# argumentcomputer/lurk-beta

Measured on AMD Instinct MI355X. Metric: MSM Mscalar-mul/s (Pallas Pedersen commitment, bases+scalars resident in HBM), higher is better.
Workload: dtype u32x8 (255-bit Montgomery, integer VALU)

## Files before the change

### lurk_beta_amd/csrc/field.cuh

```cuda
#pragma once
#include <stdint.h>

#if defined(__HIPCC__)
#define LURK_HD __host__ __device__ __forceinline__
#else
#define LURK_HD inline
#endif

namespace lurk {

struct PallasFp {
    static constexpr int ID = 0;
    static constexpr int NBITS = 255;
    static constexpr uint32_t INV = 0xffffffffu;
    LURK_HD static constexpr uint32_t mod(int i) {
        constexpr uint32_t m[8] = {0x00000001u, 0x992d30edu, 0x094cf91bu, 0x224698fcu, 0x00000000u, 0x00000000u, 0x00000000u, 0x40000000u};
        return m[i];
    }
    LURK_HD static constexpr uint32_t r(int i) {
        constexpr uint32_t m[8] = {0xfffffffdu, 0x34786d38u, 0xe41914adu, 0x992c350bu, 0xffffffffu, 0xffffffffu, 0xffffffffu, 0x3fffffffu};
        return m[i];
    }
    LURK_HD static constexpr uint32_t r2(int i) {
        constexpr uint32_t m[8] = {0x0000000fu, 0x8c78ecb3u, 0x8b0de0e7u, 0xd7d30dbdu, 0xc3c95d18u, 0x7797a99bu, 0x7b9cb714u, 0x096d41afu};
        return m[i];
    }
    LURK_HD static constexpr uint32_t w32(int i) {
        constexpr uint32_t m[8] = {0xbad6dbf0u, 0xa28db849u, 0xd3b539dfu, 0x9083cd03u, 0x9dc8448eu, 0xfba6b9cau, 0x7b89c6dau, 0x3ec92874u};
        return m[i];
    }
};

struct PallasFq {
    static constexpr int ID = 1;
    static constexpr int NBITS = 255;
    static constexpr uint32_t INV = 0xffffffffu;
    LURK_HD static constexpr uint32_t mod(int i) {
        constexpr uint32_t m[8] = {0x00000001u, 0x8c46eb21u, 0x0994a8ddu, 0x224698fcu, 0x00000000u, 0x00000000u, 0x00000000u, 0x40000000u};
        return m[i];
    }
    LURK_HD static constexpr uint32_t r(int i) {
        constexpr uint32_t m[8] = {0xfffffffdu, 0x5b2b3e9cu, 0xe3420567u, 0x992c350bu, 0xffffffffu, 0xffffffffu, 0xffffffffu, 0x3fffffffu};
        return m[i];
    }
    LURK_HD static constexpr uint32_t r2(int i) {
        constexpr uint32_t m[8] = {0x0000000fu, 0xfc9678ffu, 0x891a16e3u, 0x67bb433du, 0x04ccf590u, 0x7fae2310u, 0x7ccfdaa9u, 0x096d41afu};
        return m[i];
    }
    LURK_HD static constexpr uint32_t w32(int i) {
        constexpr uint32_t m[8] = {0x8c9942deu, 0x21807742u, 0x21b60494u, 0xcc495789u, 0xb2efbee2u, 0xac2e5d27u, 0x7f2db056u, 0x0b79fa89u};
        return m[i];
    }
};

struct Bn254Fr {
    static constexpr int ID = 2;
    static constexpr int NBITS = 254;
    static constexpr uint32_t INV = 0xefffffffu;
    LURK_HD static constexpr uint32_t mod(int i) {
        constexpr uint32_t m[8] = {0xf0000001u, 0x43e1f593u, 0x79b97091u, 0x2833e848u, 0x8181585du, 0xb85045b6u, 0xe131a029u, 0x30644e72u};
        return m[i];
    }
    LURK_HD static constexpr uint32_t r(int i) {
        constexpr uint32_t m[8] = {0x4ffffffbu, 0xac96341cu, 0x9f60cd29u, 0x36fc7695u, 0x7879462eu, 0x666ea36fu, 0x9a07df2fu, 0x0e0a77c1u};
        return m[i];
    }
    LURK_HD static constexpr uint32_t r2(int i) {
        constexpr uint32_t m[8] = {0xae216da7u, 0x1bb8e645u, 0xe35c59e3u, 0x53fe3ab1u, 0x53bb8085u, 0x8c49833du, 0x7f4e44a5u, 0x0216d0b1u};
        return m[i];
    }
    LURK_HD static constexpr uint32_t w32(int i) { return 0; }
};

struct Bn254Fq {
    static constexpr int ID = 3;
    static constexpr int NBITS = 254;
    static constexpr uint32_t INV = 0xe4866389u;
    LURK_HD static constexpr uint32_t mod(int i) {
        constexpr uint32_t m[8] = {0xd87cfd47u, 0x3c208c16u, 0x6871ca8du, 0x97816a91u, 0x8181585du, 0xb85045b6u, 0xe131a029u, 0x30644e72u};
        return m[i];
    }
    LURK_HD static constexpr uint32_t r(int i) {
        constexpr uint32_t m[8] = {0xc58f0d9du, 0xd35d438du, 0xf5c70b3du, 0x0a78eb28u, 0x7879462cu, 0x666ea36fu, 0x9a07df2fu, 0x0e0a77c1u};
        return m[i];
    }
    LURK_HD static constexpr uint32_t r2(int i) {
        constexpr uint32_t m[8] = {0x538afa89u, 0xf32cfc5bu, 0xd44501fbu, 0xb5e71911u, 0x0a417ff6u, 0x47ab1effu, 0xcab8351fu, 0x06d89f71u};
        return m[i];
    }
    LURK_HD static constexpr uint32_t w32(int i) { return 0; }
};

template <class P>
struct alignas(16) Fe {
    uint32_t l[8];
};

template <class P>
LURK_HD Fe<P> fe_zero() {
    Fe<P> z;
#pragma unroll
    for (int i = 0; i < 8; i++) z.l[i] = 0;
    return z;
}
template <class P>
LURK_HD Fe<P> fe_one() {
    Fe<P> z;
#pragma unroll
    for (int i = 0; i < 8; i++) z.l[i] = P::r(i);
    return z;
}
template <class P>
LURK_HD Fe<P> fe_r2() {
    Fe<P> z;
#pragma unroll
    for (int i = 0; i < 8; i++) z.l[i] = P::r2(i);
    return z;
}
template <class P>
LURK_HD bool fe_is_zero(const Fe<P>& a) {
    uint32_t o = 0;
#pragma unroll
    for (int i = 0; i < 8; i++) o |= a.l[i];
    return o == 0;
}
template <class P>
LURK_HD bool fe_eq(const Fe<P>& a, const Fe<P>& b) {
    uint32_t o = 0;
#pragma unroll
    for (int i = 0; i < 8; i++) o |= a.l[i] ^ b.l[i];
    return o == 0;
}

LURK_HD uint32_t addc32(uint32_t a, uint32_t b, uint32_t& carry) {
#if defined(__HIP_DEVICE_COMPILE__)
    unsigned c;
    uint32_t r = __builtin_addc(a, b, carry, &c);
    carry = c;
    return r;
#else
    uint64_t x = (uint64_t)a + b + carry;
    carry = (uint32_t)(x >> 32);
    return (uint32_t)x;
#endif
}
LURK_HD uint32_t subb32(uint32_t a, uint32_t b, uint32_t& borrow) {
#if defined(__HIP_DEVICE_COMPILE__)
    unsigned c;
    uint32_t r = __builtin_subc(a, b, borrow, &c);
    borrow = c;
    return r;
#else
    uint64_t x = (uint64_t)a - b - borrow;
    borrow = (uint32_t)(x >> 63);
    return (uint32_t)x;
#endif
}

#if defined(LURK_FE_CHECK) && !defined(__HIP_DEVICE_COMPILE__)
#define FE_CHECKS_ACTIVE 1
}
#include <cstdio>
#include <cstdlib>
namespace lurk {
template <class P>
inline void fe_assert_canonical(const uint32_t* v, const char* what) {
    for (int i = 7; i >= 0; i--) {
        if (v[i] < P::mod(i)) return;
        if (v[i] > P::mod(i)) break;
    }
    fprintf(stderr, "Fe contract violated: %s operand >= p\n", what);
    abort();
}
#define FE_ASSERT_CANONICAL(P, x, what) fe_assert_canonical<P>((x).l, what)
#else
#define FE_CHECKS_ACTIVE 0
#define FE_ASSERT_CANONICAL(P, x, what) ((void)0)
#endif

template <class P>
LURK_HD void fe_cond_sub(uint32_t* t) {
    uint32_t d[8];
    uint32_t borrow = 0;
#pragma unroll
    for (int i = 0; i < 8; i++) d[i] = subb32(t[i], P::mod(i), borrow);
#pragma unroll
    for (int i = 0; i < 8; i++) t[i] = borrow ? t[i] : d[i];
}

template <class P>
LURK_HD Fe<P> fe_add(const Fe<P>& a, const Fe<P>& b) {
    FE_ASSERT_CANONICAL(P, a, "fe_add");
    FE_ASSERT_CANONICAL(P, b, "fe_add");
    Fe<P> r;
    uint32_t c = 0;
#pragma unroll
    for (int i = 0; i < 8; i++) r.l[i] = addc32(a.l[i], b.l[i], c);
    fe_cond_sub<P>(r.l);
    return r;
}
template <class P>
LURK_HD Fe<P> fe_sub(const Fe<P>& a, const Fe<P>& b) {
    FE_ASSERT_CANONICAL(P, a, "fe_sub");
    FE_ASSERT_CANONICAL(P, b, "fe_sub");
    Fe<P> r;
    uint32_t borrow = 0;
#pragma unroll
    for (int i = 0; i < 8; i++) r.l[i] = subb32(a.l[i], b.l[i], borrow);
    uint32_t mask = 0u - borrow, c = 0;
#pragma unroll
    for (int i = 0; i < 8; i++) r.l[i] = addc32(r.l[i], P::mod(i) & mask, c);
    return r;
}
template <class P>
LURK_HD Fe<P> fe_neg(const Fe<P>& a) {
    return fe_sub<P>(fe_zero<P>(), a);
}
template <class P>
LURK_HD Fe<P> fe_dbl(const Fe<P>& a) {
    return fe_add<P>(a, a);
}

template <class P>
LURK_HD Fe<P> fe_mul_cios(const Fe<P>& a, const Fe<P>& b) {
    uint32_t t[8];
#pragma unroll
    for (int i = 0; i < 8; i++) t[i] = 0;
#pragma unroll
    for (int i = 0; i < 8; i++) {
        uint32_t bi = b.l[i];
        uint64_t acc = (uint64_t)a.l[0] * bi + t[0];
        uint32_t m = (uint32_t)acc * P::INV;
        uint64_t red = (uint64_t)m * P::mod(0) + (uint32_t)acc;
        uint32_t c1 = (uint32_t)(acc >> 32), c2 = (uint32_t)(red >> 32);
#pragma unroll
        for (int j = 1; j < 8; j++) {
            acc = (uint64_t)a.l[j] * bi + t[j] + c1;
            c1 = (uint32_t)(acc >> 32);
            red = (uint64_t)m * P::mod(j) + (uint32_t)acc + c2;
            c2 = (uint32_t)(red >> 32);
            t[j - 1] = (uint32_t)red;
        }
        t[7] = c1 + c2;
    }
    fe_cond_sub<P>(t);
    Fe<P> r;
#pragma unroll
    for (int i = 0; i < 8; i++) r.l[i] = t[i];
    return r;
}

LURK_HD void mad_c(uint64_t& acc, uint64_t& carry, uint32_t a, uint32_t b) {
#if defined(__HIP_DEVICE_COMPILE__)
    asm volatile("v_mad_u64_u32 %0, %1, %2, %3, %0" : "+v"(acc), "=s"(carry) : "v"(a), "v"(b));
#else
    uint64_t p = (uint64_t)a * b;
    acc += p;
    carry = (acc < p) ? 1u : 0u;
#endif
}
LURK_HD void mad_ck(uint64_t& acc, uint64_t& carry, uint32_t a, uint32_t k) {
#if defined(__HIP_DEVICE_COMPILE__)
    asm volatile("v_mad_u64_u32 %0, %1, %2, %3, %0" : "+v"(acc), "=s"(carry) : "v"(a), "s"(k));
#else
    mad_c(acc, carry, a, k);
#endif
}
LURK_HD void column_fence() {
#if defined(__HIP_DEVICE_COMPILE__)
    asm volatile("s_nop 1");
#endif
}
LURK_HD void fold_carry(uint32_t& hi, uint64_t carry) {
#if defined(__HIP_DEVICE_COMPILE__)
    asm volatile("v_addc_co_u32_e64 %0, vcc, 0, %0, %1" : "+v"(hi) : "s"(carry) : "vcc");
#else
    hi += (uint32_t)carry;
#endif
}

template <class P>
LURK_HD Fe<P> fe_mul_fips(const Fe<P>& a, const Fe<P>& b) {
    uint32_t m[8], t[8];
    uint64_t lo = 0;
    uint32_t hi = 0;
#pragma unroll
    for (int k = 0; k < 16; k++) {
        uint64_t cm[16];
        int n = 0;
        const int i0 = k < 8 ? 0 : k - 7, i1 = k < 8 ? k : 7;
#pragma unroll
        for (int i = i0; i <= i1; i++) mad_c(lo, cm[n++], a.l[i], b.l[k - i]);
#pragma unroll
        for (int i = i0; i <= (k < 8 ? k - 1 : 7); i++)
            if (P::mod(k - i) != 0) mad_ck(lo, cm[n++], m[i], P::mod(k - i));
        bool carry_in_one = false;
        uint32_t c0 = 0;
        if (k < 8) {
            c0 = (uint32_t)lo;
            m[k] = c0 * P::INV;
            if (P::mod(0) == 1 && P::INV == 0xffffffffu) {
                carry_in_one = true;
            } else {
                mad_ck(lo, cm[n++], m[k], P::mod(0));
            }
        }
        column_fence();
#pragma unroll
        for (int i = 0; i < n; i++) fold_carry(hi, cm[i]);
        if (k >= 8) t[k - 8] = (uint32_t)lo;
        lo = (lo >> 32) | ((uint64_t)hi << 32);
        if (carry_in_one) lo += (c0 != 0 ? 1u : 0u);
        hi = 0;
    }
    fe_cond_sub<P>(t);
    Fe<P> r;
#pragma unroll
    for (int i = 0; i < 8; i++) r.l[i] = t[i];
    return r;
}

#if !defined(__HIP_DEVICE_COMPILE__) && defined(__SIZEOF_INT128__)
template <class P>
inline Fe<P> fe_mul_host64(const Fe<P>& a, const Fe<P>& b) {
    typedef unsigned __int128 u128;
    uint64_t x[4], y[4], m[4], t[6] = {0, 0, 0, 0, 0, 0};
    for (int i = 0; i < 4; i++) {
        x[i] = (uint64_t)a.l[2 * i] | ((uint64_t)a.l[2 * i + 1] << 32);
        y[i] = (uint64_t)b.l[2 * i] | ((uint64_t)b.l[2 * i + 1] << 32);
        m[i] = (uint64_t)P::mod(2 * i) | ((uint64_t)P::mod(2 * i + 1) << 32);
    }
    uint64_t inv32 = P::INV;
    uint64_t ninv = (uint64_t)0 - inv32;
    ninv *= 2 - m[0] * ninv;
    const uint64_t inv = (uint64_t)0 - ninv;
    for (int i = 0; i < 4; i++) {
        u128 c = 0;
        for (int j = 0; j < 4; j++) {
            c += (u128)x[j] * y[i] + t[j];
            t[j] = (uint64_t)c;
            c >>= 64;
        }
        c += t[4];
        t[4] = (uint64_t)c;
        t[5] = (uint64_t)(c >> 64);
        uint64_t q = t[0] * inv;
        c = ((u128)q * m[0] + t[0]) >> 64;
        for (int j = 1; j < 4; j++) {
            c += (u128)q * m[j] + t[j];
            t[j - 1] = (uint64_t)c;
            c >>= 64;
        }
        c += t[4];
        t[3] = (uint64_t)c;
        t[4] = t[5] + (uint64_t)(c >> 64);
    }
    uint64_t d[4];
    u128 br = 0;
    for (int i = 0; i < 4; i++) {
        u128 v = (u128)t[i] - m[i] - br;
        d[i] = (uint64_t)v;
        br = (v >> 64) & 1;
    }
    bool ge = t[4] != 0 || br == 0;
    Fe<P> r;
    for (int i = 0; i < 4; i++) {
        uint64_t v = ge ? d[i] : t[i];
        r.l[2 * i] = (uint32_t)v;
        r.l[2 * i + 1] = (uint32_t)(v >> 32);
    }
    return r;
}
#define LURK_HAVE_HOST64 1
#endif

#ifndef LURK_MUL_IMPL
#define LURK_MUL_IMPL 2
#endif
}
#include "field_mul_asm.cuh"
#include "field_mul_asm_bn254fq.cuh"
namespace lurk {
template <class P>
LURK_HD Fe<P> fe_mul_inline(const Fe<P>& a, const Fe<P>& b) {
#if LURK_MUL_IMPL == 0
    return fe_mul_cios<P>(a, b);
#elif LURK_MUL_IMPL == 2 && defined(__HIP_DEVICE_COMPILE__)
    return fe_mul_asm<P>(a, b);
#elif !defined(__HIP_DEVICE_COMPILE__) && defined(LURK_HAVE_HOST64) && !defined(LURK_HOST_PORTABLE_MUL)
    return fe_mul_host64<P>(a, b);
#else
    return fe_mul_fips<P>(a, b);
#endif
}
#if defined(__HIPCC__)
template <class P>
__device__ __attribute__((noinline)) Fe<P> fe_mul_call(Fe<P> a, Fe<P> b) {
    return fe_mul_inline<P>(a, b);
}
#endif
template <class P>
LURK_HD Fe<P> fe_mul(const Fe<P>& a, const Fe<P>& b) {
    FE_ASSERT_CANONICAL(P, a, "fe_mul");
    FE_ASSERT_CANONICAL(P, b, "fe_mul");
#if defined(__HIP_DEVICE_COMPILE__) && !defined(LURK_MUL_FORCE_INLINE)
    return fe_mul_call<P>(a, b);
#else
    return fe_mul_inline<P>(a, b);
#endif
}
template <class P>
LURK_HD void fe_cond_sub2(uint32_t* t) {
    uint32_t d[8];
    uint32_t borrow = 0;
#pragma unroll
    for (int i = 0; i < 8; i++) {
        uint32_t twop = (P::mod(i) << 1) | (i ? (P::mod(i - 1) >> 31) : 0u);
        d[i] = subb32(t[i], twop, borrow);
    }
#pragma unroll
    for (int i = 0; i < 8; i++) t[i] = borrow ? t[i] : d[i];
}

template <class P>
struct DotAcc {
    uint64_t col[15];
    uint32_t h[15];
};
template <class P>
LURK_HD void dot_init(DotAcc<P>& A) {
#pragma unroll
    for (int k = 0; k < 15; k++) {
        A.col[k] = 0;
        A.h[k] = 0;
    }
}
template <class P>
LURK_HD void dot_mac(DotAcc<P>& A, const Fe<P>& a, const Fe<P>& b) {
#pragma unroll
    for (int j = 0; j < 8; j++) {
        uint64_t cm[8];
#pragma unroll
        for (int l = 0; l < 8; l++) mad_c(A.col[j + l], cm[l], a.l[j], b.l[l]);
        column_fence();
#pragma unroll
        for (int l = 0; l < 8; l++) fold_carry(A.h[j + l], cm[l]);
    }
}
template <class P>
LURK_HD void fe_redc16_portable(uint32_t* t, const uint32_t* vin) {
    uint32_t v[17];
#pragma unroll
    for (int i = 0; i < 16; i++) v[i] = vin[i];
    v[16] = 0;
#pragma unroll
    for (int k = 0; k < 8; k++) {
        uint32_t m = v[k] * P::INV;
        uint64_t c = 0;
#pragma unroll
        for (int j = 0; j < 8; j++) {
            uint64_t x = (uint64_t)m * P::mod(j) + v[k + j] + c;
            v[k + j] = (uint32_t)x;
            c = x >> 32;
        }
#pragma unroll
        for (int j = k + 8; j < 17; j++) {
            uint64_t x = (uint64_t)v[j] + c;
            v[j] = (uint32_t)x;
            c = x >> 32;
        }
    }
#pragma unroll
    for (int i = 0; i < 8; i++) t[i] = v[8 + i];
}

template <class P, int T>
LURK_HD Fe<P> dot_finish(const DotAcc<P>& A) {
    uint32_t x[16], v[16];
    uint32_t c1 = 0, c2 = 0;
#pragma unroll
    for (int k = 0; k < 16; k++) {
        uint32_t lo = k < 15 ? (uint32_t)A.col[k] : 0u;
        uint32_t hi = k >= 1 ? (uint32_t)(A.col[k - 1] >> 32) : 0u;
        x[k] = addc32(lo, hi, c1);
    }
#pragma unroll
    for (int k = 0; k < 16; k++) v[k] = addc32(x[k], k >= 2 ? A.h[k - 2] : 0u, c2);
    uint32_t t[8];
#if defined(__HIP_DEVICE_COMPILE__) && LURK_MUL_IMPL == 2
    fe_redc16_asm<P>(t, v);
#else
    fe_redc16_portable<P>(t, v);
#endif
    if (T > 3) fe_cond_sub2<P>(t);
    fe_cond_sub<P>(t);
    Fe<P> r;
#pragma unroll
    for (int i = 0; i < 8; i++) r.l[i] = t[i];
    return r;
}

template <class P>
LURK_HD Fe<P> fe_sqr(const Fe<P>& a) {
    return fe_mul<P>(a, a);
}

template <class P>
LURK_HD Fe<P> fe_to_mont(const Fe<P>& a) {
    return fe_mul<P>(a, fe_r2<P>());
}
template <class P>
LURK_HD Fe<P> fe_from_mont(const Fe<P>& a) {
    Fe<P> one = fe_zero<P>();
    one.l[0] = 1;
    return fe_mul<P>(a, one);
}
template <class P>
LURK_HD Fe<P> fe_from_u64(uint64_t v) {
    Fe<P> x = fe_zero<P>();
    x.l[0] = (uint32_t)v;
    x.l[1] = (uint32_t)(v >> 32);
    return fe_to_mont<P>(x);
}

template <class P>
LURK_HD Fe<P> fe_pow(const Fe<P>& a, const uint32_t* e) {
    Fe<P> acc = fe_one<P>();
    for (int i = 255; i >= 0; i--) {
        acc = fe_sqr<P>(acc);
        if ((e[i >> 5] >> (i & 31)) & 1) acc = fe_mul<P>(acc, a);
    }
    return acc;
}
#if !defined(__HIP_DEVICE_COMPILE__)
namespace host_inv {
struct U256 {
    uint64_t w[4];
};
inline bool is_one(const U256& a) { return a.w[0] == 1 && (a.w[1] | a.w[2] | a.w[3]) == 0; }
inline bool ge(const U256& a, const U256& b) {
    for (int i = 3; i >= 0; i--)
        if (a.w[i] != b.w[i]) return a.w[i] > b.w[i];
    return true;
}
inline uint64_t add(U256& a, const U256& b) {
    unsigned __int128 c = 0;
    for (int i = 0; i < 4; i++) {
        c += (unsigned __int128)a.w[i] + b.w[i];
        a.w[i] = (uint64_t)c;
        c >>= 64;
    }
    return (uint64_t)c;
}
inline void sub(U256& a, const U256& b) {
    uint64_t borrow = 0;
    for (int i = 0; i < 4; i++) {
        const uint64_t bi = b.w[i], t = a.w[i] - bi, t2 = t - borrow;
        borrow = (uint64_t)(a.w[i] < bi) | (uint64_t)(t < borrow);
        a.w[i] = t2;
    }
}
inline void shr1(U256& a, uint64_t top) {
    a.w[0] = (a.w[0] >> 1) | (a.w[1] << 63);
    a.w[1] = (a.w[1] >> 1) | (a.w[2] << 63);
    a.w[2] = (a.w[2] >> 1) | (a.w[3] << 63);
    a.w[3] = (a.w[3] >> 1) | (top << 63);
}
inline void halve_mod(U256& x, const U256& p) {
    if (x.w[0] & 1) {
        const uint64_t c = add(x, p);
        shr1(x, c);
    } else {
        shr1(x, 0);
    }
}
inline void sub_mod(U256& x, const U256& y, const U256& p) {
    if (ge(x, y)) {
        sub(x, y);
    } else {
        U256 t = p;
        sub(t, y);
        add(x, t);
    }
}
inline bool is_zero(const U256& a) { return (a.w[0] | a.w[1] | a.w[2] | a.w[3]) == 0; }
inline U256 inverse(U256 u, const U256& p) {
    while (ge(u, p)) sub(u, p);
    if (is_zero(u)) return u;
    U256 v = p, x1 = {{1, 0, 0, 0}}, x2 = {{0, 0, 0, 0}};
    while (!is_one(u) && !is_one(v)) {
        while (!(u.w[0] & 1)) {
            shr1(u, 0);
            halve_mod(x1, p);
        }
        while (!(v.w[0] & 1)) {
            shr1(v, 0);
            halve_mod(x2, p);
        }
        if (ge(u, v)) {
            sub(u, v);
            sub_mod(x1, x2, p);
        } else {
            sub(v, u);
            sub_mod(x2, x1, p);
        }
    }
    return is_one(u) ? x1 : x2;
}
}
#endif

template <class P>
LURK_HD Fe<P> fe_inv(const Fe<P>& a) {
#if !defined(__HIP_DEVICE_COMPILE__)
    host_inv::U256 u, p;
    for (int i = 0; i < 4; i++) {
        u.w[i] = (uint64_t)a.l[2 * i] | ((uint64_t)a.l[2 * i + 1] << 32);
        p.w[i] = (uint64_t)P::mod(2 * i) | ((uint64_t)P::mod(2 * i + 1) << 32);
    }
    const host_inv::U256 x = host_inv::inverse(u, p);
    Fe<P> xi;
    for (int i = 0; i < 4; i++) {
        xi.l[2 * i] = (uint32_t)x.w[i];
        xi.l[2 * i + 1] = (uint32_t)(x.w[i] >> 32);
    }
    const Fe<P> r2 = fe_r2<P>();
    return fe_mul<P>(xi, fe_mul<P>(r2, r2));
#else
    uint32_t e[8];
    uint32_t borrow = 2;
    for (int i = 0; i < 8; i++) {
        uint64_t x = (uint64_t)P::mod(i) - borrow;
        e[i] = (uint32_t)x;
        borrow = (uint32_t)(x >> 63);
    }
    return fe_pow<P>(a, e);
#endif
}
template <class P>
LURK_HD Fe<P> fe_inv_pow(const Fe<P>& a) {
    uint32_t e[8];
    uint32_t borrow = 2;
    for (int i = 0; i < 8; i++) {
        uint64_t x = (uint64_t)P::mod(i) - borrow;
        e[i] = (uint32_t)x;
        borrow = (uint32_t)(x >> 63);
    }
    return fe_pow<P>(a, e);
}

template <class P>
LURK_HD bool fe_canonical_ge_mod(const uint32_t* v) {
    for (int i = 7; i >= 0; i--) {
        if (v[i] > P::mod(i)) return true;
        if (v[i] < P::mod(i)) return false;
    }
    return true;
}

}
```

### lurk_beta_amd/csrc/msm_core.cuh

```cuda
#pragma once
#include "curve.cuh"

namespace lurk {

constexpr int MSM_C_PLAIN = 16;
constexpr int MSM_MAX_W = 16;
constexpr int MSM_GRP = 1 << 15;
constexpr uint32_t MSM_SIGN = 0x80000000u;
constexpr int MSM_PLACEMENT_BASE = 16;

LURK_HD int msm_num_windows(int c) { return (256 + c - 1) / c; }

LURK_HD uint32_t msm_digit_step(const uint32_t* s, int w, int c, uint32_t& carry) {
    const uint32_t half = 1u << (c - 1), mask = (1u << c) - 1u;
    const int bit = w * c, limb = bit >> 5, sh = bit & 31;
    uint32_t raw = 0;
    if (limb < 8) {
        uint64_t v = s[limb];
        if (limb + 1 < 8) v |= (uint64_t)s[limb + 1] << 32;
        raw = (uint32_t)(v >> sh) & mask;
    }
    raw += carry;
    if (raw > half) {
        carry = 1;
        return ((1u << c) - raw) | MSM_SIGN;
    }
    carry = 0;
    return raw;
}

LURK_HD uint32_t msm_digit_next(uint32_t (&r)[8], int c, uint32_t& carry) {
    const uint32_t half = 1u << (c - 1), mask = (1u << c) - 1u;
    uint32_t raw = (r[0] & mask) + carry;
#pragma unroll
    for (int k = 0; k < 7; k++) r[k] = (r[k] >> c) | (r[k + 1] << (32 - c));
    r[7] >>= c;
    if (raw > half) {
        carry = 1;
        return ((1u << c) - raw) | MSM_SIGN;
    }
    carry = 0;
    return raw;
}

template <int C>
LURK_HD void msm_digits_ct(const uint32_t (&s)[8], uint32_t (&d)[(256 + C - 1) / C]) {
    constexpr int W = (256 + C - 1) / C;
    constexpr uint32_t half = 1u << (C - 1), mask = (1u << C) - 1u;
    uint32_t carry = 0;
#pragma unroll
    for (int w = 0; w < W; w++) {
        const int bit = w * C, limb = bit >> 5, sh = bit & 31;
        uint32_t raw = s[limb] >> sh;
        if (sh + C > 32 && limb + 1 < 8) raw |= s[limb + 1] << (32 - sh);
        raw = (raw & mask) + carry;
        const bool neg = raw > half;
        carry = neg ? 1u : 0u;
        d[w] = neg ? (((1u << C) - raw) | MSM_SIGN) : raw;
    }
}

LURK_HD uint32_t msm_upper_slot(const uint32_t* start, uint32_t n, uint32_t t) {
    uint32_t lo = 0, hi = n;
    while (hi - lo > 1) {
        uint32_t mid = (lo + hi) >> 1;
        if (start[mid] <= t) lo = mid;
        else hi = mid;
    }
    return lo;
}

template <class P>
LURK_HD Xyzz<P> msm_task_accumulate(const uint32_t* sorted, uint32_t first, uint32_t last, const Affine<P>* table) {
    Xyzz<P> acc = xyzz_identity<P>();
    for (uint32_t j = first; j < last; j++) {
        uint32_t e = sorted[j];
        Affine<P> q = table[e & ~MSM_SIGN];
        xyzz_madd<P>(acc, q, (e & MSM_SIGN) != 0);
    }
    return acc;
}

template <class P>
LURK_HD Xyzz<P> xyzz_dbl_n(Xyzz<P> p, int n) {
    for (int i = 0; i < n; i++) p = xyzz_dbl<P>(p);
    return p;
}

template <class P>
LURK_HD Xyzz<P> msm_planes_horner_windows(const Xyzz<P>* v, int G, int c) {
    Xyzz<P> acc = xyzz_identity<P>();
    for (int g = G - 1; g >= 0; g--) {
        const Xyzz<P>* vg = v + (size_t)g * c;
        for (int k = c - 1; k >= 0; k--) {
            acc = xyzz_dbl<P>(acc);
            if (k <= c - 2) xyzz_add<P>(acc, vg[1 + k]);
        }
        xyzz_add<P>(acc, vg[0]);
    }
    return acc;
}

}
```

### lurk_beta_amd/csrc/msm_sort.hip

```cpp
#include "msm_sort.hpp"

#include "common.hpp"
#include "msm_core.cuh"

namespace lurk {

MsmShape msm_make_shape(int c, bool precomputed, size_t npoints, size_t n, int sel) {
    MsmShape sh;
    sh.c = c;
    sh.W = msm_num_windows(c);
    sh.sel = precomputed ? sel : -1;
    sh.low_prio = 0;
    sh.G = precomputed ? (sh.sel >= 0 ? 2 : 1) : sh.W;
    sh.B = 1u << (c - 1);
    sh.NB = (uint32_t)sh.G * sh.B;
    sh.P = MSM_P_MIN;
    while (sh.P < MSM_P_MAX && (uint32_t)sh.P < sh.NB) {
        int lb = 0;
        while ((sh.NB >> lb) > (uint32_t)sh.P) lb++;
        if (lb <= MSM_LB_MAX && (double)sh.W * (double)n / sh.P <= 0.85 * (double)msm_part2_cap(lb)) break;
        sh.P *= 2;
    }
    sh.LB = 0;
    while ((sh.NB >> sh.LB) > (uint32_t)sh.P) sh.LB++;
    LURK_REQUIRE(sh.LB <= MSM_LB_MAX, "sort shape: more than 8 low key bits per partition");
    sh.tile = MSM_SORT_BLOCK;
    while (sh.tile > 64 && msm_scatter1_lds(sh.P, sh.W, sh.tile) > MSM_LDS_BYTES) sh.tile /= 2;
    sh.S = MSM_S;
    static const size_t task_target = [] { const char* e = getenv("LURK_MSM_TASK_TARGET"); long v = e ? atol(e) : 0; return v > 0 ? (size_t)v : MSM_TASK_TARGET; }();
    while (sh.S > MSM_S_MIN && (size_t)sh.W * n / sh.S < task_target) sh.S /= 2;
    sh.NG = (int)(sh.NB / MSM_GRP);
    sh.n = n;
    sh.stride = precomputed ? npoints : 0;
    return sh;
}

__device__ __forceinline__ void msm_sort_wave_prio(int low = 0) {
    if (low) __builtin_amdgcn_s_setprio(0);
    else __builtin_amdgcn_s_setprio(3);
}

__device__ __forceinline__ uint32_t msm_key(const MsmShape& sh, uint32_t w, uint32_t mag, size_t i) {
    const uint32_t space = sh.sel >= 0 ? (uint32_t)((i >> sh.sel) & 1u) : (sh.G == 1 ? 0u : w);
    return space * sh.B + mag - 1u;
}

constexpr int msm_ct_windows(int C) { return C ? (256 + C - 1) / C : 1; }

template <class SF, int C, bool MONT>
__global__ __launch_bounds__(MSM_SORT_BLOCK) void msm_hist1_kernel(const uint4* __restrict__ scalars, uint4* __restrict__ canon,
                                                                     uint32_t* __restrict__ block_hist, MsmShape sh, size_t chunk) {
    msm_sort_wave_prio(sh.low_prio);
    extern __shared__ uint32_t h[];
    for (int p = threadIdx.x; p < sh.P; p += MSM_SORT_BLOCK) h[p] = 0;
    __syncthreads();
    size_t lo = (size_t)blockIdx.x * chunk, hi = lo + chunk < sh.n ? lo + chunk : sh.n;
    size_t i = lo + threadIdx.x;
    uint4 nlo = make_uint4(0, 0, 0, 0), nhi = nlo;
    if (i < hi) { nlo = scalars[2 * i]; nhi = scalars[2 * i + 1]; }
    for (; i < hi; i += MSM_SORT_BLOCK) {
        Fe<SF> s;
        s.l[0] = nlo.x; s.l[1] = nlo.y; s.l[2] = nlo.z; s.l[3] = nlo.w;
        s.l[4] = nhi.x; s.l[5] = nhi.y; s.l[6] = nhi.z; s.l[7] = nhi.w;
        if (i + MSM_SORT_BLOCK < hi) { nlo = scalars[2 * (i + MSM_SORT_BLOCK)]; nhi = scalars[2 * (i + MSM_SORT_BLOCK) + 1]; }
        if constexpr (MONT) {
            s = fe_from_mont<SF>(s);
            canon[2 * i] = make_uint4(s.l[0], s.l[1], s.l[2], s.l[3]);
            canon[2 * i + 1] = make_uint4(s.l[4], s.l[5], s.l[6], s.l[7]);
        }
        if constexpr (C != 0) {
            uint32_t d[msm_ct_windows(C)];
            msm_digits_ct<C>(s.l, d);
#pragma unroll
            for (int w = 0; w < msm_ct_windows(C); w++) {
                const uint32_t mag = d[w] & ~MSM_SIGN;
                if (mag) atomicAdd(&h[msm_key(sh, (uint32_t)w, mag, i) >> sh.LB], 1u);
            }
        } else {
            uint32_t carry = 0;
            uint32_t r[8];
#pragma unroll
            for (int k = 0; k < 8; k++) r[k] = s.l[k];
            for (int w = 0; w < sh.W; w++) {
                uint32_t mag = msm_digit_next(r, sh.c, carry) & ~MSM_SIGN;
                if (mag) atomicAdd(&h[msm_key(sh, (uint32_t)w, mag, i) >> sh.LB], 1u);
            }
        }
    }
    __syncthreads();
    for (int p = threadIdx.x; p < sh.P; p += MSM_SORT_BLOCK) block_hist[(size_t)blockIdx.x * sh.P + p] = h[p];
}

__global__ __launch_bounds__(MSM_NB1) void msm_scan1_kernel(uint32_t* __restrict__ block_hist, uint32_t* __restrict__ part_cnt, int P) {
    msm_sort_wave_prio();
    __shared__ uint32_t sh[MSM_NB1];
    const int p = blockIdx.x, t = threadIdx.x;
    uint32_t v = block_hist[(size_t)t * P + p];
    sh[t] = v;
    __syncthreads();
    for (int off = 1; off < MSM_NB1; off <<= 1) {
        uint32_t a = t >= off ? sh[t - off] : 0;
        __syncthreads();
        sh[t] += a;
        __syncthreads();
    }
    block_hist[(size_t)t * P + p] = sh[t] - v;
    if (t == MSM_NB1 - 1) part_cnt[p] = sh[t];
}

__device__ __forceinline__ uint32_t msm_block_scan(uint32_t v, uint32_t* scr, uint32_t* total) {
    const int lane = threadIdx.x & 63, wave = threadIdx.x >> 6;
    uint32_t inc = v;
#pragma unroll
    for (int off = 1; off < 64; off <<= 1) {
        uint32_t o = __shfl_up(inc, off);
        if (lane >= off) inc += o;
    }
    if (lane == 63) scr[wave] = inc;
    __syncthreads();
    if (threadIdx.x < 64) {
        uint32_t w = threadIdx.x < MSM_SORT_BLOCK / 64 ? scr[threadIdx.x] : 0, winc = w;
#pragma unroll
        for (int off = 1; off < 16; off <<= 1) {
            uint32_t o = __shfl_up(winc, off);
            if (lane >= off) winc += o;
        }
        if (threadIdx.x < MSM_SORT_BLOCK / 64) scr[threadIdx.x] = winc - w;
        if (threadIdx.x == MSM_SORT_BLOCK / 64 - 1) scr[16] = winc;
    }
    __syncthreads();
    uint32_t ex = scr[wave] + inc - v;
    *total = scr[16];
    __syncthreads();
    return ex;
}

__global__ __launch_bounds__(MSM_SORT_BLOCK) void msm_part_start_kernel(const uint32_t* __restrict__ part_cnt, uint32_t* __restrict__ part_start,
                                                                          int P, uint32_t* __restrict__ z0, int n0, uint32_t* __restrict__ z1, int n1,
                                                                          uint32_t* __restrict__ z2, int n2) {
    msm_sort_wave_prio();
    for (int i = threadIdx.x; i < n0; i += MSM_SORT_BLOCK) z0[i] = 0;
    for (int i = threadIdx.x; i < n1; i += MSM_SORT_BLOCK) z1[i] = 0;
    for (int i = threadIdx.x; i < n2; i += MSM_SORT_BLOCK) z2[i] = 0;
    __shared__ uint32_t scr[32];
    const int PER = P / MSM_SORT_BLOCK;
    const int t = threadIdx.x;
    uint32_t c[MSM_P_PER_MAX], sum = 0;
#pragma unroll
    for (int j = 0; j < MSM_P_PER_MAX; j++) { c[j] = j < PER ? part_cnt[t * PER + j] : 0u; sum += c[j]; }
    uint32_t total;
    uint32_t run = msm_block_scan(sum, scr, &total);
#pragma unroll
    for (int j = 0; j < MSM_P_PER_MAX; j++)
        if (j < PER) { part_start[t * PER + j] = run; run += c[j]; }
    if (t == 0) part_start[P] = total;
}

#ifndef LURK_SORT_MIN_BLOCKS
#define LURK_SORT_MIN_BLOCKS 1
#endif
template <int C>
__global__ __launch_bounds__(MSM_SORT_BLOCK, LURK_SORT_MIN_BLOCKS) void msm_scatter1_kernel(const uint4* __restrict__ scalars, const uint32_t* __restrict__ block_off,
                                                                        const uint32_t* __restrict__ part_start, uint32_t* __restrict__ inter_e,
                                                                        uint8_t* __restrict__ inter_k, MsmShape sh, size_t chunk) {
    msm_sort_wave_prio(sh.low_prio);
    extern __shared__ uint32_t lds[];
    const int P = sh.P, PER = P / MSM_SORT_BLOCK;
    uint32_t* goff = lds;
    uint32_t* cnt = goff + P;
    uint32_t* start = cnt + P;
    uint32_t* scr = start + P;
    uint2* stage = reinterpret_cast<uint2*>(scr + 32);
    const int t = threadIdx.x;
    const uint32_t low_mask = (1u << sh.LB) - 1u;
    for (int p = t; p < P; p += MSM_SORT_BLOCK) {
        goff[p] = part_start[p] + block_off[(size_t)blockIdx.x * P + p];
        cnt[p] = 0;
    }
    __syncthreads();
    size_t lo = (size_t)blockIdx.x * chunk, hi = lo + chunk < sh.n ? lo + chunk : sh.n;
    for (size_t base = lo; base < hi; base += sh.tile) {
        const size_t i = base + t;
        const bool live = t < sh.tile && i < hi;
        uint32_t sl[8];
        uint32_t d[msm_ct_windows(C)];
        if (live) {
            const uint4 a = scalars[2 * i], b = scalars[2 * i + 1];
            sl[0] = a.x; sl[1] = a.y; sl[2] = a.z; sl[3] = a.w;
            sl[4] = b.x; sl[5] = b.y; sl[6] = b.z; sl[7] = b.w;
            if constexpr (C != 0) {
                msm_digits_ct<C>(sl, d);
#pragma unroll
                for (int w = 0; w < msm_ct_windows(C); w++) {
                    const uint32_t mag = d[w] & ~MSM_SIGN;
                    if (mag) atomicAdd(&cnt[msm_key(sh, (uint32_t)w, mag, i) >> sh.LB], 1u);
                }
            } else {
                uint32_t carry = 0;
                uint32_t r[8];
#pragma unroll
                for (int k = 0; k < 8; k++) r[k] = sl[k];
                for (int w = 0; w < sh.W; w++) {
                    uint32_t mag = msm_digit_next(r, sh.c, carry) & ~MSM_SIGN;
                    if (mag) atomicAdd(&cnt[msm_key(sh, (uint32_t)w, mag, i) >> sh.LB], 1u);
                }
            }
        }
        __syncthreads();
        uint32_t total;
        {
            uint32_t c[MSM_P_PER_MAX], sum = 0;
#pragma unroll
            for (int j = 0; j < MSM_P_PER_MAX; j++) { c[j] = j < PER ? cnt[t * PER + j] : 0u; sum += c[j]; }
            uint32_t run = msm_block_scan(sum, scr, &total);
#pragma unroll
            for (int j = 0; j < MSM_P_PER_MAX; j++)
                if (j < PER) { start[t * PER + j] = run; run += c[j]; cnt[t * PER + j] = 0; }
        }
        __syncthreads();
        if (live) {
            if constexpr (C != 0) {
#pragma unroll
                for (int w = 0; w < msm_ct_windows(C); w++) {
                    const uint32_t mag = d[w] & ~MSM_SIGN;
                    if (mag) {
                        const uint32_t key = msm_key(sh, (uint32_t)w, mag, i);
                        const uint32_t p = key >> sh.LB;
                        const uint32_t slot = start[p] + atomicAdd(&cnt[p], 1u);
                        stage[slot] = make_uint2(key, ((uint32_t)((size_t)w * sh.stride) + (uint32_t)i) | (d[w] & MSM_SIGN));
                    }
                }
            } else {
                uint32_t carry = 0;
                uint32_t r[8];
#pragma unroll
                for (int k = 0; k < 8; k++) r[k] = sl[k];
                for (int w = 0; w < sh.W; w++) {
                    uint32_t dg = msm_digit_next(r, sh.c, carry);
                    uint32_t mag = dg & ~MSM_SIGN;
                    if (mag) {
                        uint32_t key = msm_key(sh, (uint32_t)w, mag, i);
                        uint32_t p = key >> sh.LB;
                        uint32_t slot = start[p] + atomicAdd(&cnt[p], 1u);
                        stage[slot] = make_uint2(key, ((uint32_t)((size_t)w * sh.stride) + (uint32_t)i) | (dg & MSM_SIGN));
                    }
                }
            }
        }
        __syncthreads();
        for (uint32_t j = t; j < total; j += MSM_SORT_BLOCK) {
            const uint2 e = stage[j];
            const uint32_t p = e.x >> sh.LB;
            const uint32_t dst = goff[p] + (j - start[p]);
            inter_e[dst] = e.y;
            inter_k[dst] = (uint8_t)(e.x & low_mask);
        }
        __syncthreads();
        for (int j = 0; j < PER; j++) {
            goff[t * PER + j] += cnt[t * PER + j];
            cnt[t * PER + j] = 0;
        }
        __syncthreads();
    }
}

__global__ __launch_bounds__(MSM_SORT_BLOCK) void msm_part2_kernel(const uint32_t* __restrict__ inter_e, const uint8_t* __restrict__ inter_k,
                                                                     const uint32_t* __restrict__ part_start, uint32_t* __restrict__ sorted,
                                                                     uint32_t* __restrict__ cnt, uint32_t* __restrict__ bucket_start, MsmShape sh,
                                                                     uint32_t cap) {
    msm_sort_wave_prio(sh.low_prio);
    extern __shared__ uint32_t lds[];
    const int p = blockIdx.x, t = threadIdx.x;
    const uint32_t nbins = 1u << sh.LB;
    uint32_t* h = lds;
    uint32_t* scr = lds + nbins;
    uint32_t* stage = scr + 32;
    for (uint32_t b = t; b < nbins; b += MSM_SORT_BLOCK) h[b] = 0;
    __syncthreads();
    const uint32_t lo = part_start[p], hi = part_start[p + 1];
    const uint32_t lo4 = lo & ~3u;
    const bool staged = hi - lo <= cap;
    constexpr int U = 4;
    const uint32_t* key_words = reinterpret_cast<const uint32_t*>(inter_k);
    const uint4* entry_quads = reinterpret_cast<const uint4*>(inter_e);
    for (uint32_t base = lo4; base < hi; base += MSM_SORT_BLOCK * 4 * U) {
        uint32_t kw[U];
#pragma unroll
        for (int u = 0; u < U; u++) {
            const uint32_t e = base + (uint32_t)(u * MSM_SORT_BLOCK + t) * 4u;
            kw[u] = e < hi ? key_words[e >> 2] : 0u;
        }
#pragma unroll
        for (int u = 0; u < U; u++) {
            const uint32_t e = base + (uint32_t)(u * MSM_SORT_BLOCK + t) * 4u;
#pragma unroll
            for (int b = 0; b < 4; b++)
                if (e + b >= lo && e + b < hi) atomicAdd(&h[(kw[u] >> (8 * b)) & 0xffu], 1u);
        }
    }
    __syncthreads();
    const uint32_t per = (nbins + MSM_SORT_BLOCK - 1) / MSM_SORT_BLOCK;
    uint32_t sum = 0;
    for (uint32_t j = 0; j < per; j++) {
        uint32_t b = t * per + j;
        if (b < nbins) sum += h[b];
    }
    uint32_t total;
    uint32_t run = lo + msm_block_scan(sum, scr, &total);
    for (uint32_t j = 0; j < per; j++) {
        uint32_t b = t * per + j;
        if (b < nbins) {
            uint32_t c = h[b];
            size_t key = ((size_t)p << sh.LB) + b;
            cnt[key] = c;
            bucket_start[key] = run;
            h[b] = run;
            run += c;
        }
    }
    __syncthreads();
    for (uint32_t base = lo4; base < hi; base += MSM_SORT_BLOCK * 4 * U) {
        uint32_t kw[U];
        uint4 ev[U];
#pragma unroll
        for (int u = 0; u < U; u++) {
            const uint32_t e = base + (uint32_t)(u * MSM_SORT_BLOCK + t) * 4u;
            if (e < hi) { kw[u] = key_words[e >> 2]; ev[u] = entry_quads[e >> 2]; }
            else { kw[u] = 0u; ev[u] = make_uint4(0, 0, 0, 0); }
        }
#pragma unroll
        for (int u = 0; u < U; u++) {
            const uint32_t e = base + (uint32_t)(u * MSM_SORT_BLOCK + t) * 4u;
            const uint32_t ent[4] = {ev[u].x, ev[u].y, ev[u].z, ev[u].w};
#pragma unroll
            for (int b = 0; b < 4; b++) {
                if (e + b >= lo && e + b < hi) {
                    const uint32_t pos = atomicAdd(&h[(kw[u] >> (8 * b)) & 0xffu], 1u);
                    if (staged) stage[pos - lo] = ent[b];
                    else sorted[pos] = ent[b];
                }
            }
        }
    }
    if (staged) {
        __syncthreads();
        for (uint32_t j = t; j < hi - lo; j += MSM_SORT_BLOCK) sorted[lo + j] = stage[j];
    }
}

template <class SF, int C>
static void msm_launch_sort_c(const MsmShape& sh, const void* d_scalars, int is_mont, const MsmSortBufs& b, hipStream_t s) {
    const size_t chunk = (sh.n + MSM_NB1 - 1) / MSM_NB1;
    const size_t entries = (size_t)sh.W * sh.n;
    uint32_t* inter_e = reinterpret_cast<uint32_t*>(b.inter);
    uint8_t* inter_k = reinterpret_cast<uint8_t*>(inter_e + entries);
    allow_dynamic_lds((const void*)msm_scatter1_kernel<C>, (int)MSM_LDS_BYTES);
    allow_dynamic_lds((const void*)msm_part2_kernel, (int)MSM_LDS_BYTES);
    LURK_REQUIRE(msm_scatter1_lds(sh.P, sh.W, sh.tile) <= MSM_LDS_BYTES, "pass-1 tile does not fit the LDS");
    const uint4* canon = (const uint4*)d_scalars;
    if (is_mont) {
        hipLaunchKernelGGL((msm_hist1_kernel<SF, C, true>), dim3(MSM_NB1), dim3(MSM_SORT_BLOCK), (size_t)sh.P * 4, s, (const uint4*)d_scalars,
                           (uint4*)b.canon, b.block_hist, sh, chunk);
        canon = (const uint4*)b.canon;
    } else {
        hipLaunchKernelGGL((msm_hist1_kernel<SF, C, false>), dim3(MSM_NB1), dim3(MSM_SORT_BLOCK), (size_t)sh.P * 4, s, (const uint4*)d_scalars,
                           (uint4*)nullptr, b.block_hist, sh, chunk);
    }
    hipLaunchKernelGGL(msm_scan1_kernel, dim3(sh.P), dim3(MSM_NB1), 0, s, b.block_hist, b.part_cnt, sh.P);
    hipLaunchKernelGGL(msm_part_start_kernel, dim3(1), dim3(MSM_SORT_BLOCK), 0, s, b.part_cnt, b.part_start, sh.P, b.zero[0], b.zero_n[0], b.zero[1],
                       b.zero_n[1], b.zero[2], b.zero_n[2]);
    hipLaunchKernelGGL((msm_scatter1_kernel<C>), dim3(MSM_NB1), dim3(MSM_SORT_BLOCK), msm_scatter1_lds(sh.P, sh.W, sh.tile), s, canon, b.block_hist,
                       b.part_start, inter_e, inter_k, sh, chunk);
    hipLaunchKernelGGL(msm_part2_kernel, dim3(sh.P), dim3(MSM_SORT_BLOCK), MSM_LDS_BYTES, s, inter_e, inter_k, b.part_start, b.sorted, b.cnt,
                       b.bucket_start, sh, (uint32_t)msm_part2_cap(sh.LB));
}

template <class SF>
void msm_launch_sort(const MsmShape& sh, const void* d_scalars, int is_mont, const MsmSortBufs& b, hipStream_t s) {
    if (sh.c == 20) msm_launch_sort_c<SF, 20>(sh, d_scalars, is_mont, b, s);
    else if (sh.c == 16) msm_launch_sort_c<SF, 16>(sh, d_scalars, is_mont, b, s);
    else msm_launch_sort_c<SF, 0>(sh, d_scalars, is_mont, b, s);
}
template void msm_launch_sort<PallasFp>(const MsmShape&, const void*, int, const MsmSortBufs&, hipStream_t);
template void msm_launch_sort<PallasFq>(const MsmShape&, const void*, int, const MsmSortBufs&, hipStream_t);

void msm_launch_sort_canonical(const MsmShape& sh, const void* d_scalars, const MsmSortBufs& b, hipStream_t s) {
    msm_launch_sort<PallasFp>(sh, d_scalars, 0, b, s);
}

}
```

Before: 993.4.

## Trim sort-kernel register pressure and use DPP wave scans

The sort kernels now compute signed digits on the fly instead of holding a per-window digit array in registers. The Montgomery-to-canonical conversion uses a dedicated word-by-word reduction instead of a full multiply by one, and the scalar prefetch is moved after that conversion. The block scan swaps shuffle-based steps for DPP row operations, and several loops gain unroll pragmas plus 32-bit indexing. Together these aim to cut VGPR use and instruction count in the sorting pre-pass, at the cost of recomputing digits twice in the scatter kernel.

```diff
diff --git a/lurk_beta_amd/csrc/field.cuh b/lurk_beta_amd/csrc/field.cuh
--- a/lurk_beta_amd/csrc/field.cuh
+++ b/lurk_beta_amd/csrc/field.cuh
@@ -516,6 +516,30 @@
     return fe_mul<P>(a, one);
 }
 template <class P>
+LURK_HD Fe<P> fe_from_mont_words(const Fe<P>& a) {
+    uint32_t t[8];
+#pragma unroll
+    for (int i = 0; i < 8; i++) t[i] = a.l[i];
+#pragma unroll
+    for (int i = 0; i < 8; i++) {
+        const uint32_t m = t[0] * P::INV;
+        uint64_t red = (uint64_t)m * P::mod(0) + t[0];
+        uint32_t c = (uint32_t)(red >> 32);
+#pragma unroll
+        for (int j = 1; j < 8; j++) {
+            red = (uint64_t)m * P::mod(j) + t[j] + c;
+            c = (uint32_t)(red >> 32);
+            t[j - 1] = (uint32_t)red;
+        }
+        t[7] = c;
+    }
+    fe_cond_sub<P>(t);
+    Fe<P> r;
+#pragma unroll
+    for (int i = 0; i < 8; i++) r.l[i] = t[i];
+    return r;
+}
+template <class P>
 LURK_HD Fe<P> fe_from_u64(uint64_t v) {
     Fe<P> x = fe_zero<P>();
     x.l[0] = (uint32_t)v;
diff --git a/lurk_beta_amd/csrc/msm_core.cuh b/lurk_beta_amd/csrc/msm_core.cuh
--- a/lurk_beta_amd/csrc/msm_core.cuh
+++ b/lurk_beta_amd/csrc/msm_core.cuh
@@ -44,20 +44,23 @@
 }
 
 template <int C>
+LURK_HD uint32_t msm_digit_ct_next(const uint32_t (&s)[8], int w, uint32_t& carry) {
+    constexpr uint32_t half = 1u << (C - 1), mask = (1u << C) - 1u;
+    const int bit = w * C, limb = bit >> 5, sh = bit & 31;
+    uint32_t raw = s[limb] >> sh;
+    if (sh + C > 32 && limb + 1 < 8) raw |= s[limb + 1] << (32 - sh);
+    raw = (raw & mask) + carry;
+    const bool neg = raw > half;
+    carry = neg ? 1u : 0u;
+    return neg ? (((1u << C) - raw) | MSM_SIGN) : raw;
+}
+
+template <int C>
 LURK_HD void msm_digits_ct(const uint32_t (&s)[8], uint32_t (&d)[(256 + C - 1) / C]) {
     constexpr int W = (256 + C - 1) / C;
-    constexpr uint32_t half = 1u << (C - 1), mask = (1u << C) - 1u;
     uint32_t carry = 0;
 #pragma unroll
-    for (int w = 0; w < W; w++) {
-        const int bit = w * C, limb = bit >> 5, sh = bit & 31;
-        uint32_t raw = s[limb] >> sh;
-        if (sh + C > 32 && limb + 1 < 8) raw |= s[limb + 1] << (32 - sh);
-        raw = (raw & mask) + carry;
-        const bool neg = raw > half;
-        carry = neg ? 1u : 0u;
-        d[w] = neg ? (((1u << C) - raw) | MSM_SIGN) : raw;
-    }
+    for (int w = 0; w < W; w++) d[w] = msm_digit_ct_next<C>(s, w, carry);
 }
 
 LURK_HD uint32_t msm_upper_slot(const uint32_t* start, uint32_t n, uint32_t t) {
diff --git a/lurk_beta_amd/csrc/msm_sort.hip b/lurk_beta_amd/csrc/msm_sort.hip
--- a/lurk_beta_amd/csrc/msm_sort.hip
+++ b/lurk_beta_amd/csrc/msm_sort.hip
@@ -52,6 +52,7 @@
                                                                      uint32_t* __restrict__ block_hist, MsmShape sh, size_t chunk) {
     msm_sort_wave_prio(sh.low_prio);
     extern __shared__ uint32_t h[];
+#pragma unroll 1
     for (int p = threadIdx.x; p < sh.P; p += MSM_SORT_BLOCK) h[p] = 0;
     __syncthreads();
     size_t lo = (size_t)blockIdx.x * chunk, hi = lo + chunk < sh.n ? lo + chunk : sh.n;
@@ -62,18 +63,17 @@
         Fe<SF> s;
         s.l[0] = nlo.x; s.l[1] = nlo.y; s.l[2] = nlo.z; s.l[3] = nlo.w;
         s.l[4] = nhi.x; s.l[5] = nhi.y; s.l[6] = nhi.z; s.l[7] = nhi.w;
-        if (i + MSM_SORT_BLOCK < hi) { nlo = scalars[2 * (i + MSM_SORT_BLOCK)]; nhi = scalars[2 * (i + MSM_SORT_BLOCK) + 1]; }
         if constexpr (MONT) {
-            s = fe_from_mont<SF>(s);
+            s = fe_from_mont_words<SF>(s);
             canon[2 * i] = make_uint4(s.l[0], s.l[1], s.l[2], s.l[3]);
             canon[2 * i + 1] = make_uint4(s.l[4], s.l[5], s.l[6], s.l[7]);
         }
+        if (i + MSM_SORT_BLOCK < hi) { nlo = scalars[2 * (i + MSM_SORT_BLOCK)]; nhi = scalars[2 * (i + MSM_SORT_BLOCK) + 1]; }
         if constexpr (C != 0) {
-            uint32_t d[msm_ct_windows(C)];
-            msm_digits_ct<C>(s.l, d);
+            uint32_t carry = 0;
 #pragma unroll
             for (int w = 0; w < msm_ct_windows(C); w++) {
-                const uint32_t mag = d[w] & ~MSM_SIGN;
+                const uint32_t mag = msm_digit_ct_next<C>(s.l, w, carry) & ~MSM_SIGN;
                 if (mag) atomicAdd(&h[msm_key(sh, (uint32_t)w, mag, i) >> sh.LB], 1u);
             }
         } else {
@@ -88,6 +88,7 @@
         }
     }
     __syncthreads();
+#pragma unroll 1
     for (int p = threadIdx.x; p < sh.P; p += MSM_SORT_BLOCK) block_hist[(size_t)blockIdx.x * sh.P + p] = h[p];
 }
 
@@ -108,23 +109,27 @@
     if (t == MSM_NB1 - 1) part_cnt[p] = sh[t];
 }
 
+__device__ __forceinline__ uint32_t msm_wave_scan(uint32_t v, bool rows = true) {
+    v += (uint32_t)__builtin_amdgcn_update_dpp(0, (int)v, 0x111, 0xf, 0xf, false);
+    v += (uint32_t)__builtin_amdgcn_update_dpp(0, (int)v, 0x112, 0xf, 0xf, false);
+    v += (uint32_t)__builtin_amdgcn_update_dpp(0, (int)v, 0x114, 0xf, 0xf, false);
+    v += (uint32_t)__builtin_amdgcn_update_dpp(0, (int)v, 0x118, 0xf, 0xf, false);
+    if (rows) {
+        v += (uint32_t)__builtin_amdgcn_update_dpp(0, (int)v, 0x142, 0xa, 0xf, false);
+        v += (uint32_t)__builtin_amdgcn_update_dpp(0, (int)v, 0x143, 0xc, 0xf, false);
+    }
+    return v;
+}
+
 __device__ __forceinline__ uint32_t msm_block_scan(uint32_t v, uint32_t* scr, uint32_t* total) {
-    const int lane = threadIdx.x & 63, wave = threadIdx.x >> 6;
-    uint32_t inc = v;
-#pragma unroll
-    for (int off = 1; off < 64; off <<= 1) {
-        uint32_t o = __shfl_up(inc, off);
-        if (lane >= off) inc += o;
-    }
+    static_assert(MSM_SORT_BLOCK / 64 <= 16, "the wave totals are scanned inside one row of 16 lanes");
+    const uint32_t lane = threadIdx.x & 63, wave = threadIdx.x >> 6;
+    const uint32_t inc = msm_wave_scan(v);
     if (lane == 63) scr[wave] = inc;
     __syncthreads();
     if (threadIdx.x < 64) {
-        uint32_t w = threadIdx.x < MSM_SORT_BLOCK / 64 ? scr[threadIdx.x] : 0, winc = w;
-#pragma unroll
-        for (int off = 1; off < 16; off <<= 1) {
-            uint32_t o = __shfl_up(winc, off);
-            if (lane >= off) winc += o;
-        }
+        const uint32_t w = threadIdx.x < MSM_SORT_BLOCK / 64 ? scr[threadIdx.x] : 0;
+        const uint32_t winc = msm_wave_scan(w, false);
         if (threadIdx.x < MSM_SORT_BLOCK / 64) scr[threadIdx.x] = winc - w;
         if (threadIdx.x == MSM_SORT_BLOCK / 64 - 1) scr[16] = winc;
     }
@@ -165,34 +170,34 @@
                                                                         uint8_t* __restrict__ inter_k, MsmShape sh, size_t chunk) {
     msm_sort_wave_prio(sh.low_prio);
     extern __shared__ uint32_t lds[];
-    const int P = sh.P, PER = P / MSM_SORT_BLOCK;
+    const uint32_t P = (uint32_t)sh.P, PER = P / MSM_SORT_BLOCK;
     uint32_t* goff = lds;
     uint32_t* cnt = goff + P;
     uint32_t* start = cnt + P;
     uint32_t* scr = start + P;
     uint2* stage = reinterpret_cast<uint2*>(scr + 32);
-    const int t = threadIdx.x;
+    const uint32_t t = threadIdx.x;
     const uint32_t low_mask = (1u << sh.LB) - 1u;
-    for (int p = t; p < P; p += MSM_SORT_BLOCK) {
+#pragma unroll 1
+    for (uint32_t p = t; p < P; p += MSM_SORT_BLOCK) {
         goff[p] = part_start[p] + block_off[(size_t)blockIdx.x * P + p];
         cnt[p] = 0;
     }
     __syncthreads();
-    size_t lo = (size_t)blockIdx.x * chunk, hi = lo + chunk < sh.n ? lo + chunk : sh.n;
-    for (size_t base = lo; base < hi; base += sh.tile) {
-        const size_t i = base + t;
-        const bool live = t < sh.tile && i < hi;
+    const uint32_t lo = (uint32_t)(blockIdx.x * chunk), hi = (size_t)lo + chunk < sh.n ? lo + (uint32_t)chunk : (uint32_t)sh.n;
+    for (uint32_t base = lo; base < hi; base += (uint32_t)sh.tile) {
+        const uint32_t i = base + t;
+        const bool live = t < (uint32_t)sh.tile && i < hi;
         uint32_t sl[8];
-        uint32_t d[msm_ct_windows(C)];
         if (live) {
-            const uint4 a = scalars[2 * i], b = scalars[2 * i + 1];
+            const uint4 a = scalars[2 * (size_t)i], b = scalars[2 * (size_t)i + 1];
             sl[0] = a.x; sl[1] = a.y; sl[2] = a.z; sl[3] = a.w;
             sl[4] = b.x; sl[5] = b.y; sl[6] = b.z; sl[7] = b.w;
             if constexpr (C != 0) {
-                msm_digits_ct<C>(sl, d);
+                uint32_t carry = 0;
 #pragma unroll
                 for (int w = 0; w < msm_ct_windows(C); w++) {
-                    const uint32_t mag = d[w] & ~MSM_SIGN;
+                    const uint32_t mag = msm_digit_ct_next<C>(sl, w, carry) & ~MSM_SIGN;
                     if (mag) atomicAdd(&cnt[msm_key(sh, (uint32_t)w, mag, i) >> sh.LB], 1u);
                 }
             } else {
@@ -209,25 +214,31 @@
         __syncthreads();
         uint32_t total;
         {
-            uint32_t c[MSM_P_PER_MAX], sum = 0;
-#pragma unroll
-            for (int j = 0; j < MSM_P_PER_MAX; j++) { c[j] = j < PER ? cnt[t * PER + j] : 0u; sum += c[j]; }
+            uint32_t sum = 0;
+#pragma unroll 1
+            for (uint32_t j = 0; j < PER; j++) sum += cnt[t * PER + j];
             uint32_t run = msm_block_scan(sum, scr, &total);
-#pragma unroll
-            for (int j = 0; j < MSM_P_PER_MAX; j++)
-                if (j < PER) { start[t * PER + j] = run; run += c[j]; cnt[t * PER + j] = 0; }
+#pragma unroll 1
+            for (uint32_t j = 0; j < PER; j++) {
+                const uint32_t c = cnt[t * PER + j];
+                start[t * PER + j] = run;
+                cnt[t * PER + j] = 0;
+                run += c;
+            }
         }
         __syncthreads();
         if (live) {
             if constexpr (C != 0) {
+                uint32_t carry = 0;
 #pragma unroll
                 for (int w = 0; w < msm_ct_windows(C); w++) {
-                    const uint32_t mag = d[w] & ~MSM_SIGN;
+                    const uint32_t dg = msm_digit_ct_next<C>(sl, w, carry);
+                    const uint32_t mag = dg & ~MSM_SIGN;
                     if (mag) {
                         const uint32_t key = msm_key(sh, (uint32_t)w, mag, i);
                         const uint32_t p = key >> sh.LB;
                         const uint32_t slot = start[p] + atomicAdd(&cnt[p], 1u);
-                        stage[slot] = make_uint2(key, ((uint32_t)((size_t)w * sh.stride) + (uint32_t)i) | (d[w] & MSM_SIGN));
+                        stage[slot] = make_uint2(key, ((uint32_t)((size_t)w * sh.stride) + i) | (dg & MSM_SIGN));
                     }
                 }
             } else {
@@ -242,12 +253,13 @@
                         uint32_t key = msm_key(sh, (uint32_t)w, mag, i);
                         uint32_t p = key >> sh.LB;
                         uint32_t slot = start[p] + atomicAdd(&cnt[p], 1u);
-                        stage[slot] = make_uint2(key, ((uint32_t)((size_t)w * sh.stride) + (uint32_t)i) | (dg & MSM_SIGN));
+                        stage[slot] = make_uint2(key, ((uint32_t)((size_t)w * sh.stride) + i) | (dg & MSM_SIGN));
                     }
                 }
             }
         }
         __syncthreads();
+#pragma clang loop vectorize(disable) interleave(disable) unroll_count(2)
         for (uint32_t j = t; j < total; j += MSM_SORT_BLOCK) {
             const uint2 e = stage[j];
             const uint32_t p = e.x >> sh.LB;
@@ -256,7 +268,8 @@
             inter_k[dst] = (uint8_t)(e.x & low_mask);
         }
         __syncthreads();
-        for (int j = 0; j < PER; j++) {
+#pragma unroll 1
+        for (uint32_t j = 0; j < PER; j++) {
             goff[t * PER + j] += cnt[t * PER + j];
             cnt[t * PER + j] = 0;
         }
@@ -275,6 +288,7 @@
     uint32_t* h = lds;
     uint32_t* scr = lds + nbins;
     uint32_t* stage = scr + 32;
+#pragma unroll 1
     for (uint32_t b = t; b < nbins; b += MSM_SORT_BLOCK) h[b] = 0;
     __syncthreads();
     const uint32_t lo = part_start[p], hi = part_start[p + 1];
@@ -301,12 +315,14 @@
     __syncthreads();
     const uint32_t per = (nbins + MSM_SORT_BLOCK - 1) / MSM_SORT_BLOCK;
     uint32_t sum = 0;
+#pragma unroll 1
     for (uint32_t j = 0; j < per; j++) {
         uint32_t b = t * per + j;
         if (b < nbins) sum += h[b];
     }
     uint32_t total;
     uint32_t run = lo + msm_block_scan(sum, scr, &total);
+#pragma unroll 1
     for (uint32_t j = 0; j < per; j++) {
         uint32_t b = t * per + j;
         if (b < nbins) {
@@ -344,6 +360,7 @@
     }
     if (staged) {
         __syncthreads();
+#pragma clang loop vectorize(disable) interleave(disable) unroll_count(4)
         for (uint32_t j = t; j < hi - lo; j += MSM_SORT_BLOCK) sorted[lo + j] = stage[j];
     }
 }
```

Measured after the change: 993.9, median of 2. Within noise of the previous version (+0.1%).
